# siyi-wind/MDViT

Hardware: NVIDIA B200
Metric: mdvit_train_images_per_sec (higher is better)
Workload: dtype bf16

## Files before the change

include/mdvit_b200.h:

```cpp
#ifndef MDVIT_B200_H
#define MDVIT_B200_H
#include <stdint.h>

#ifdef __cplusplus
extern "C" {
#endif

#define MDV_ACT_NONE 0
#define MDV_ACT_GELU 1
#define MDV_ACT_RELU 2
#define MDV_ACT_HSWISH 3

int mdv_version(void);
long long mdv_launch_count(void);
int mdv_set_pdl(int enabled);

typedef struct MdvGemmEpi {
    const float* bias;
    const float* residual;
    const void* mul_gelu_grad;
    void* out_preact;
    void* out;
    const float* rowscale;
    const void* rng;
// ... 16 lines not shown

int mdv_conv3_gemm(const void* x, int x_f32, int ldx, const void* Wm, int ldw, int B, int H, int W, int Cin, int N, int flip,
                   const MdvGemmEpi* epi, void* stream);

int mdv_conv3_wgrad(const void* dz_bf16, int ldz, const void* x_bf16, int ldx, int B, int H, int W, int Cin, int P, float* dWm, int ldc,
                    void* stream);

int mdv_gemm_tn(const void* A, int lda, const void* B, int ldb, int R, int P, int Q, float* C, int ldc, void* stream);

int mdv_mlp_supported(int C, int hidden);
int mdv_mlp_fwd(const void* a_bf16, const void* w1_bf16, const float* b1, const void* w2_bf16, const float* b2, const float* residual,
                float* out, void* hact_out, void* u_out, int M, int C, int hidden, float drop_p, const void* rng, uint32_t drop_stream1,
                uint32_t drop_stream2, const float* rowscale, int rows_per_scale, void* stream);
int mdv_mlp_bwd(const void* dy_bf16, const void* w2t_bf16, const void* u_bf16, const void* w1t_bf16, void* du_out, float* dx_out,
                float* colsum1, int M, int C, int hidden, void* stream);

int mdv_gemm_tune(int force_bn, int force_stages, int force_split);
int mdv_gemm_force_pair(int mode);

int mdv_layernorm_fwd(const float* x, const float* gamma, const float* beta, float eps, void* y_bf16, float* mean,
                      float* rstd, int M, int C, void* stream);
int mdv_layernorm_bwd(const float* dy, const float* x, const float* mean, const float* rstd, const float* gamma,
                      const float* dres, float* dx, void* dx_masked_bf16, const float* rowscale, int rows_per_scale,
                      float drop_p, const void* rng, uint32_t drop_stream, float* dgamma, float* dbeta,
                      float* dbias_masked , int M, int C, void* stream);

#define MDV_MAX_GROUPS 8
typedef struct MdvPtrTable {
    void* p[MDV_MAX_GROUPS];
} MdvPtrTable;

int mdv_layernorm_fwd_gp(const float* x, MdvPtrTable gamma, MdvPtrTable beta, float eps, void* y_bf16, float* mean, float* rstd,
                         int G, int Mg, int C, void* stream);
int mdv_layernorm_bwd_gp(const float* dy, const float* x, const float* mean, const float* rstd, MdvPtrTable gamma,
                         const float* dres, float* dx, void* dx_masked_bf16, const float* rowscale, int rows_per_scale,
                         float drop_p, const void* rng, uint32_t drop_stream, MdvPtrTable dgamma, MdvPtrTable dbeta,
                         float* dbias_masked, int G, int Mg, int C, void* stream);
int mdv_bn_train_fwd_gp(const float* z, int G, int Mg, int C, float eps, float momentum, MdvPtrTable running_mean,
                        MdvPtrTable running_var, MdvPtrTable num_batches_tracked, MdvPtrTable gamma, MdvPtrTable beta, int act,
                        float* mean, float* rstd, void* y, int y_bf16, void* ws, void* stream);
int mdv_bn_act_bwd_gp(const float* dy, const float* z, const float* mean, const float* rstd, MdvPtrTable gamma, MdvPtrTable beta,
                      int act, void* dz, int dz_bf16, MdvPtrTable dgamma, MdvPtrTable dbeta, int G, int Mg, int C, void* ws,
                      void* stream);

int mdv_bn_stats(const float* z, int M, int C, float eps, float momentum, int training, float* running_mean,
                 float* running_var, long long* num_batches_tracked, float* mean, float* rstd, void* ws, void* stream);
int mdv_bn_fold(const float* gamma, const float* beta, const float* running_mean, const float* running_var, const float* conv_bias,
                float eps, float* scale, float* shift, int C, void* stream);
int mdv_bn_act_fwd(const float* z, const float* mean, const float* rstd, const float* gamma, const float* beta, int act,
                   void* y, int y_bf16, int M, int C, void* stream);
int mdv_bn_act_bwd(const float* dy, const float* z, const float* mean, const float* rstd, const float* gamma,
                   const float* beta, int act, void* dz, int dz_bf16, float* dgamma, float* dbeta, int M, int C, void* ws,
                   void* stream);
int mdv_bn_train_fwd_grouped(const float* z, int G, int Mg, int C, float eps, float momentum, float* running_mean, float* running_var,
                             long long* num_batches_tracked, const float* gamma, const float* beta, int act, float* mean, float* rstd,
                             void* y, int y_bf16, void* ws, void* stream);
int mdv_bn_act_bwd_grouped(const float* dy, const float* z, const float* mean, const float* rstd, const float* gamma, const float* beta,
                           int act, void* dz, int dz_bf16, float* dgamma, float* dbeta, int G, int Mg, int C, void* ws, void* stream);
int mdv_bn_act_bwd_rank1(const float* dlog, const float* wrow, int rows_per_sample, float drop_p, const void* rng,
                         uint32_t drop_stream, const float* z, const float* mean, const float* rstd, const float* gamma,
                         const float* beta, int act, void* dz, int dz_bf16, float* dgamma, float* dbeta, int M, int C, void* ws,
                         void* stream);

int mdv_dwconv3(const float* in, const float* w, const float* bias, void* out, int out_bf16, int B, int Hi, int Wi, int Ho,
                int Wo, int C, int stride, int transposed, int residual, void* stream);
int mdv_dwconv3_wgrad(const float* dy, const float* x, float* dw, float* db, int B, int Hi, int Wi, int Ho, int Wo, int C,
                      int stride, void* stream);
int mdv_gconv2_fwd(const float* skip, const float* up, const float* w, void* out, int out_bf16, int B, int H, int W, int C,
                   void* stream);
int mdv_gconv2_bwd(const float* dout, const float* skip, const float* up, const float* w, float* dskip, float* dup, float* dw,
                   int B, int H, int W, int C, void* stream);
int mdv_im2col3(const void* in, int in_bf16, void* col, int col_bf16, int B, int Hi, int Wi, int Ho, int Wo, int C, int stride,
                int ldc, void* stream);
int mdv_im2col_stem(const float* img_nchw, void* col, int col_bf16, int B, int Hi, int Wi, void* stream);
int mdv_col2im3(const float* dcol, float* dx, int B, int Hi, int Wi, int Ho, int Wo, int C, int stride, int ldc, void* stream);
int mdv_im2col3_dil(const void* in, int in_bf16, void* col, int B, int H, int W, int C, int dil, int ldc, void* stream);
int mdv_col2im3_dil(const float* dcol, float* dx, int B, int H, int W, int C, int dil, int ldc, int accumulate, void* stream);
int mdv_upsample_fwd(const void* in, int in_bf16, int ld_in, void* out, int out_bf16, int ld_out, int B, int Hi, int Wi, int Ho,
                     int Wo, int C, void* stream);
int mdv_upsample_add(float* out, int ld_out, int B, int Ho, int Wo, int C, const float* in0, int H0, int W0, const float* in1, int H1,
                     int W1, const float* in2, int H2, int W2, void* stream);
int mdv_upsample_bwd(const void* dout, int dout_bf16, int ld_out, float* din, int ld_in, int B, int Hi, int Wi, int Ho, int Wo,
                     int C, float* ws, void* stream);

long long mdv_attn_stats_floats(int B, int C, int heads);
long long mdv_attn_ws_floats(int B, int C, int heads);
int mdv_attn_fwd(const void* qkv_bf16, const float* gate, const float* crpe_w3, const float* crpe_b3, const float* crpe_w5,
                 const float* crpe_b5, const float* crpe_w7, const float* crpe_b7, float* stats, float* ws, void* out_bf16,
                 void* e_out_bf16 , int B, int H, int W, int C, int heads,
                 void* stream);
int mdv_attn_bwd(const void* qkv_bf16, const void* dy_bf16, const void* y_bf16, const void* e_bf16, const float* gate, const float* crpe_w3,
                 const float* crpe_b3, const float* crpe_w5, const float* crpe_b5, const float* crpe_w7, const float* crpe_b7,
                 const float* stats, void* dqkv_bf16, float* dgate, float* dcrpe_w3, float* dcrpe_b3, float* dcrpe_w5,
                 float* dcrpe_b5, float* dcrpe_w7, float* dcrpe_b7,
                 float* dbias_qkv , float* ws, int B,
                 int H, int W, int C, int heads,
                 void* stream);
int mdv_da_gate_fwd(const float* label, const float* w1, const float* b1, const float* w2, const float* b2, float* hid_out,
                    float* gate, int B, int nd, int hid, int C, int heads, void* stream);
int mdv_da_gate_bwd(const float* label, const float* w2, const float* hid_in, const float* gate, const float* dgate, float* dw1,
                    float* db1, float* dw2, float* db2, float* ws , int B, int nd, int hid, int C, int heads,
                    void* stream);

int mdv_sdpa_fwd(const void* qkv_bf16, const float* gate, void* out_bf16, float* lse, int B, int N, int C, int heads, float scale,
                 void* stream);
int mdv_sdpa_bwd(const void* qkv_bf16, const float* gate, const void* out_bf16, const float* lse, const void* dout_bf16,
                 void* dqkv_bf16, float* dgate, int B, int N, int C, int heads, float scale, void* stream);

int mdv_im2col_k(const float* in, int in_nchw, void* col, int col_bf16, int B, int Hi, int Wi, int Ho, int Wo, int C, int k, int stride,
                 int pad, int ldc, void* stream);
int mdv_col2im_k(const float* dcol, float* dx, int B, int Hi, int Wi, int Ho, int Wo, int C, int k, int stride, int pad, int ldc,
                 void* stream);
int mdv_maxpool3s2_fwd(const float* in, float* out, void* tap_u8, int B, int Hi, int Wi, int C, void* stream);
int mdv_maxpool3s2_bwd(const float* dout, const void* tap_u8, float* din, int B, int Hi, int Wi, int C, void* stream);
int mdv_add_act(const float* a, const float* b, float* out, long long n, int act, void* stream);
int mdv_relu_bwd(const float* dy, const float* y, float* dx, long long n, void* stream);
int mdv_resize_ac_fwd(const float* in, float* out, int B, int Hi, int Wi, int Ho, int Wo, int C, void* stream);
int mdv_resize_ac_bwd(const float* dout, float* din, int B, int Hi, int Wi, int Ho, int Wo, int C, void* stream);
int mdv_gate_cat_fwd(const float* g, const float* pgate, const float* x, const float* vgate, const float* bp, float* out, int M, int C1,
                     int C2, int C3, int rows_per_sample, void* stream);
int mdv_gate_cat_bwd(const float* dout, const float* g, const float* pgate, const float* x, const float* vgate, float* dg, float* dp, float* dx,
                     float* dv, float* dbp, int M, int C1, int C2, int C3, int rows_per_sample, void* stream);
int mdv_channel_pool_fwd(const float* x, float* out, void* arg_i32, int M, int C, void* stream);
int mdv_channel_pool_bwd(const float* dout, const void* arg_i32, float* dx, int M, int C, void* stream);
int mdv_dropout2d(const float* x, float* out, int M, int C, int rows_per_sample, float p, const void* rng, uint32_t drop_stream, void* stream);
int mdv_structure_weit(const float* mask, float* weit, float* ws, int B, int H, int W, void* stream);
int mdv_structure_loss_fwd(const float* pred, const float* mask, const float* weit, void* sums, float* loss, int B, int HW, void* stream);
int mdv_structure_loss_bwd(const float* pred, const float* mask, const float* weit, const void* sums, const float* gout, float coef,
                           float* dpred, int B, int HW, int accumulate, void* stream);

int mdv_rowdot_fwd(const void* x, int x_bf16, const float* w, const float* bias, float* out, int M, int C, int rows_per_sample,
                   float drop_p, const void* rng, uint32_t drop_stream, void* stream);
int mdv_rowdot_bwd(const float* dlog, const void* x, int x_bf16, const float* w, float* dx, float* dw, float* db, int M, int C,
                   int rows_per_sample, float drop_p, const void* rng, uint32_t drop_stream, void* stream);
int mdv_colsum(const void* x, int x_bf16, int ld, float* out, int M, int C, void* stream);
int mdv_cast_bf16(const float* in, int ld_in, void* out_bf16, int ld_out, long long M, int C, const float* rowscale,
                  int rows_per_scale, float drop_p, const void* rng, uint32_t drop_stream, float* colsum, void* stream);
int mdv_add_f32(const void* in, int in_bf16, int ld_in, float* out, int ld_out, long long M, int C, int accumulate, void* stream);
typedef struct MdvMatmulDesc {
    const float* A;
    const float* B;
    float* C;
    const float* u;
    const float* v;
    int lda, ldb, ldc, M, N, K, trans_a, trans_b, accumulate, pad_;
} MdvMatmulDesc;
int mdv_matmul_f32_grouped(const MdvMatmulDesc* descs, int n, void* stream);
int mdv_prep_weight(const float* src, void* dst, int R, int Cc, int ld, int mode, int cin, void* stream);
typedef struct MdvPrepDesc {
    const float* src;
    void* dst;
    int rows, cols, ld, mode, cin, pad_;
} MdvPrepDesc;
int mdv_prep_weights_batched(const MdvPrepDesc* descs_dev, int n, void* stream);
int mdv_unperm_conv_grad(const float* g, int ld, float* dw, int R, int cin, void* stream);

int mdv_loss_sums(const float* out, const float* aux, const void* label, int label_u8, void* sums, long long n, void* stream);
int mdv_loss_finalize(const void* sums, double n_total, float* losses , void* stream);
int mdv_loss_bwd(const float* out, const float* aux, const void* label, int label_u8, const void* sums, double n_total,
                 const float* coef, float* dout, float* daux, long long n, void* stream);

int mdv_seg_counts(const float* logits, const void* label, int label_u8, void* counts, long long n, void* stream);

int mdv_adamw(float* p, const float* g, float* m, float* v, void* hyper, long long n, void* stream);
int mdv_rng_bump(void* rng , void* stream);
int mdv_droppath_scale(float* scale, int B, float p, const void* rng, uint32_t drop_stream, void* stream);
// ... 6 lines not shown
```

mdvit_b200/csrc/conv.cu:

```cuda
#include "../../include/mdvit_b200.h"
#include "common.cuh"

namespace {

typedef int idx_t;

__device__ __forceinline__ float4 ld4(const float* p) { return *reinterpret_cast<const float4*>(p); }
__device__ __forceinline__ void st4(float* p, float4 v) { *reinterpret_cast<float4*>(p) = v; }
__device__ __forceinline__ void st4(bf16* p, float4 v) {
    *reinterpret_cast<uint2*>(p) = make_uint2(f2_to_bf2(v.x, v.y), f2_to_bf2(v.z, v.w));
}
__device__ __forceinline__ float4 ld4(const bf16* p) {
    uint2 u = *reinterpret_cast<const uint2*>(p);
    float2 a = bf2_to_f2(u.x), b = bf2_to_f2(u.y);
    return make_float4(a.x, a.y, b.x, b.y);
}
__device__ __forceinline__ void fma4(float4& a, const float4& w, const float4& x) {
    a.x += w.x * x.x; a.y += w.y * x.y; a.z += w.z * x.z; a.w += w.w * x.w;
}

template <typename TO, int STRIDE>
__global__ void __launch_bounds__(256) dwconv3_kernel(const float* __restrict__ in, const float* __restrict__ w,
                                                       const float* __restrict__ bias, TO* __restrict__ out, int B, int Hi,
                                                       int Wi, int Ho, int Wo, int C, int stride_rt, int transposed, int residual) {
// ... 866 lines not shown
        const int xa = S * xi - S / 2, ya = S * yi - S / 2;
        float acc[8] = {0.f, 0.f, 0.f, 0.f, 0.f, 0.f, 0.f, 0.f};
#pragma unroll
        for (int r = 0; r < 2 * S; ++r) {
            const int y = min(max(ya + r, 0), Ho - 1);
            const float wy = wty[yi * 2 * S + r];
            const bf16* prow = dout + ((size_t)(b * Ho + y) * Wo) * ld_out + c;
            uint4 v[2 * S];
#pragma unroll
            for (int k = 0; k < 2 * S; ++k) v[k] = *reinterpret_cast<const uint4*>(prow + (size_t)min(max(xa + k, 0), Wo - 1) * ld_out);
#pragma unroll
            for (int k = 0; k < 2 * S; ++k) fma8(acc, wy * wtab[xi * 2 * S + k], v[k]);
        }
        float* o = din + (size_t)pix * ld_in + c;
        st4(o, make_float4(acc[0], acc[1], acc[2], acc[3]));
        st4(o + 4, make_float4(acc[4], acc[5], acc[6], acc[7]));
    }
}

template <int S>
__global__ void __launch_bounds__(256) upsample_bwd_int1_kernel(const float* __restrict__ dout, float* __restrict__ din, int B, int Hi,
                                                                 int Wi) {
    MDV_PDL_SYNC();
    extern __shared__ float wtab[];
    float* wty = wtab + Wi * 2 * S;
    upsample_wtab<S>(wtab, Wi);
    upsample_wtab<S>(wty, Hi);
    __syncthreads();
    const int Ho = Hi * S, Wo = Wi * S;
    const int total = B * Hi * Wi;
    for (int idx = blockIdx.x * blockDim.x + threadIdx.x; idx < total; idx += gridDim.x * blockDim.x) {
        const int xi = idx % Wi;
        const int yi = (idx / Wi) % Hi;
        const int b = idx / (Wi * Hi);
        const int xa = S * xi - S / 2, ya = S * yi - S / 2;
        float wx[2 * S];
#pragma unroll
        for (int k = 0; k < 2 * S; ++k) wx[k] = wtab[xi * 2 * S + k];
        float acc = 0.f;
#pragma unroll 2
        for (int r = 0; r < 2 * S; ++r) {
            const int y = min(max(ya + r, 0), Ho - 1);
            const float* prow = dout + (size_t)(b * Ho + y) * Wo;
            float rs = 0.f;
#pragma unroll
            for (int k = 0; k < 2 * S; ++k) rs = fmaf(wx[k], __ldg(prow + min(max(xa + k, 0), Wo - 1)), rs);
            acc = fmaf(wty[yi * 2 * S + r], rs, acc);
        }
        din[idx] = acc;
    }
}

template <int S>
__global__ void __launch_bounds__(256) upsample_bwd_v_kernel(const float* __restrict__ tmp, float* __restrict__ din, int ld_in, int B,
                                                              int Hi, int Wi, int C) {
    MDV_PDL_SYNC();
    const int Ho = Hi * S;
    const int cvn = C >> 2;
    const float sc = 1.f / S;
    const int total = B * Hi * Wi * cvn;
    for (int idx = blockIdx.x * blockDim.x + threadIdx.x; idx < total; idx += gridDim.x * blockDim.x) {
        const int c = (idx % cvn) * 4;
        const int pix = idx / cvn;
        const int xi = pix % Wi;
        const int yi = (pix / Wi) % Hi;
        const int b = pix / (Wi * Hi);
        const int ya = S * yi - S / 2;
        float4 acc = make_float4(0.f, 0.f, 0.f, 0.f);
#pragma unroll
        for (int r = 0; r < 2 * S; ++r) {
            const int y = ya + r;
            if (y < 0 || y >= Ho) continue;
            int y0, y1;
            float ly;
            bil_src(y, sc, Hi, y0, y1, ly);
            const float wgt = (y0 == yi ? 1.f - ly : 0.f) + (y1 == yi ? ly : 0.f);
            const float4 v = ld4(tmp + ((size_t)(b * Ho + y) * Wi + xi) * C + c);
            acc.x += wgt * v.x; acc.y += wgt * v.y; acc.z += wgt * v.z; acc.w += wgt * v.w;
        }
        st4(din + (size_t)pix * ld_in + c, acc);
    }
}

inline int grid_for(long long total_threads) {
    long long b = (total_threads + 255) / 256;
    const long long cap = (long long)MDV_NUM_SMS * 16;
    return (int)(b < cap ? (b > 0 ? b : 1) : cap);
}
inline bool fits_i32(long long n) { return n > 0 && n < 0x7fffffffLL; }
inline int pix_per_block_for(long long npix, int col_blocks) {
    int want = (8 * MDV_NUM_SMS) / (col_blocks > 0 ? col_blocks : 1);
    if (want < 1) want = 1;
    long long ppb = (npix + want - 1) / want;
    if (ppb < 64) ppb = 64;
    return (int)ppb;
}

}

extern "C" int mdv_dwconv3(const float* in, const float* w, const float* bias, void* out, int out_bf16, int B, int Hi, int Wi,
                           int Ho, int Wo, int C, int stride, int transposed, int residual, void* stream) {
    if (!in || !w || !out || (C & 3) || B <= 0) return MDV_ERR_ARG;
    if (!fits_i32((long long)B * (Hi > Ho ? Hi : Ho) * (Wi > Wo ? Wi : Wo) * C)) return MDV_ERR_UNSUPPORTED;
    const long long total = (long long)B * Ho * Wo * (C / 4);
    const size_t smem = (size_t)10 * C * sizeof(float);
    cudaStream_t st = (cudaStream_t)stream;
    if (stride == 1 && Hi == Ho && Wi == Wo) {
        int seg = Hi >= 64 ? 16 : (Hi >= 16 ? 8 : Hi);
        while (seg < Hi && seg < 64 && (long long)mdv_cdiv((long long)Wi * C, 1024) * mdv_cdiv(Hi, 2 * seg) * B >= 4 * MDV_NUM_SMS) seg *= 2;
        dim3 grid(mdv_cdiv((long long)Wi * C, 1024), mdv_cdiv(Hi, seg), B);
        if (out_bf16) mdv_launch(dwconv3_s1_kernel<bf16>, dim3(grid), dim3(256), 0, st, in, w, bias, (bf16*)out, Hi, Wi, C, transposed, residual, seg);
        else mdv_launch(dwconv3_s1_kernel<float>, dim3(grid), dim3(256), 0, st, in, w, bias, (float*)out, Hi, Wi, C, transposed, residual, seg);
        MDV_CHECK_LAUNCH();
        return MDV_OK;
    }
#define MDV_DW(TO_, S_) mdv_launch((dwconv3_kernel<TO_, S_>), dim3(grid_for(total)), dim3(256), smem, st, in, w, bias, (TO_*)out, B, Hi, Wi, Ho, Wo, C, stride, transposed, residual)
    if (out_bf16) {
        if (stride == 2) MDV_DW(bf16, 2); else if (stride == 1) MDV_DW(bf16, 1); else MDV_DW(bf16, 0);
    } else {
        if (stride == 2) MDV_DW(float, 2); else if (stride == 1) MDV_DW(float, 1); else MDV_DW(float, 0);
    }
#undef MDV_DW
    MDV_CHECK_LAUNCH();
    return MDV_OK;
}

extern "C" int mdv_dwconv3_wgrad(const float* dy, const float* x, float* dw, float* db, int B, int Hi, int Wi, int Ho, int Wo,
                                 int C, int stride, void* stream) {
    if (!dy || !x || !dw || B <= 0) return MDV_ERR_ARG;
    if (!fits_i32((long long)B * Hi * Wi * C)) return MDV_ERR_UNSUPPORTED;
    if (stride == 1 && Hi == Ho && Wi == Wo && !(C & 3) && C * 40 <= 48 * 1024) {
        int seg = Hi >= 64 ? 16 : (Hi >= 16 ? 8 : Hi);
        while (seg < Hi && seg < 64 && (long long)mdv_cdiv((long long)Wi * C, 1024) * mdv_cdiv(Hi, 2 * seg) * B >= 4 * MDV_NUM_SMS) seg *= 2;
        dim3 grid(mdv_cdiv((long long)Wi * C, 1024), mdv_cdiv(Hi, seg), B);
        mdv_launch(dwconv3_s1_wgrad_kernel, dim3(grid), dim3(256), (size_t)C * 10 * sizeof(float), (cudaStream_t)stream, dy, x, dw, db, Hi, Wi, C, seg);
        MDV_CHECK_LAUNCH();
        return MDV_OK;
    }
    const long long npix = (long long)B * Ho * Wo;
    const int cb = mdv_cdiv(C, 32);
    const int ppb = pix_per_block_for(npix, cb);
    dim3 grid(cb, mdv_cdiv(npix, ppb));
    mdv_launch(dwconv3_wgrad_kernel, dim3(grid), dim3(256), 0, (cudaStream_t)stream, dy, x, dw, db, B, Hi, Wi, Ho, Wo, C, stride, ppb);
    MDV_CHECK_LAUNCH();
    return MDV_OK;
}

extern "C" int mdv_gconv2_fwd(const float* skip, const float* up, const float* w, void* out, int out_bf16, int B, int H, int W, int C,
                              void* stream) {
    if (!skip || !up || !w || !out || (C & 3)) return MDV_ERR_ARG;
    if (!fits_i32((long long)B * H * W * C)) return MDV_ERR_UNSUPPORTED;
    {
        const int seg = H >= 64 ? 16 : (H >= 16 ? 8 : H);
        if (out_bf16)
            mdv_launch(gconv2_s_fwd_kernel<bf16>, dim3(mdv_cdiv(W * (C / 2), 256), mdv_cdiv(H, seg), B), dim3(256), 0, (cudaStream_t)stream, skip, up, w,
                       (bf16*)out, H, W, C, seg);
        else
            mdv_launch(gconv2_s_fwd_kernel<float>, dim3(mdv_cdiv(W * (C / 2), 256), mdv_cdiv(H, seg), B), dim3(256), 0, (cudaStream_t)stream, skip, up, w,
                       (float*)out, H, W, C, seg);
    }
    MDV_CHECK_LAUNCH();
    return MDV_OK;
}

extern "C" int mdv_gconv2_bwd(const float* dout, const float* skip, const float* up, const float* w, float* dskip, float* dup,
                              float* dw, int B, int H, int W, int C, void* stream) {
// ... 116 lines not shown
                                int H1, int W1, const float* in2, int H2, int W2, void* stream) {
    if (!out || B <= 0 || Ho <= 0 || Wo <= 0 || C <= 0 || (C & 3) || (ld_out & 3) || ld_out < C || (reinterpret_cast<uintptr_t>(out) & 15))
        return MDV_ERR_ARG;
    UpIn3 in = {};
    int n = 0;
    const float* ps[3] = {in0, in1, in2};
    const int hs[3] = {H0, H1, H2}, ws[3] = {W0, W1, W2};
    for (int k = 0; k < 3; ++k) {
        if (!ps[k]) continue;
        if (hs[k] <= 0 || ws[k] <= 0 || (reinterpret_cast<uintptr_t>(ps[k]) & 15)) return MDV_ERR_ARG;
        if (!fits_i32((long long)B * hs[k] * ws[k] * C)) return MDV_ERR_UNSUPPORTED;
        in.p[n] = ps[k]; in.H[n] = hs[k]; in.W[n] = ws[k];
        ++n;
    }
    if (!n) return MDV_OK;
    const int seg = Ho >= 64 ? 32 : Ho;
    mdv_launch(upsample_add_kernel, dim3(mdv_cdiv(Wo * (C / 4), 256), mdv_cdiv(Ho, seg), B), dim3(256), 0, (cudaStream_t)stream, in, n, out,
               ld_out, Ho, Wo, C, seg);
    MDV_CHECK_LAUNCH();
    return MDV_OK;
}

extern "C" int mdv_upsample_bwd(const void* dout, int dout_bf16, int ld_out, float* din, int ld_in, int B, int Hi, int Wi, int Ho,
                                int Wo, int C, float* ws, void* stream) {
    if (!dout || !din || B <= 0) return MDV_ERR_ARG;
    if (!fits_i32((long long)B * Ho * Wo * (ld_out > C ? ld_out : C))) return MDV_ERR_UNSUPPORTED;
    cudaStream_t st = (cudaStream_t)stream;
    if (C == 1) {
        if (dout_bf16) return MDV_ERR_UNSUPPORTED;
        const int S1 = (Ho % Hi == 0 && Wo % Wi == 0 && Ho / Hi == Wo / Wi) ? Ho / Hi : 0;
        if ((S1 == 2 || S1 == 4 || S1 == 8) && (size_t)(Wi + Hi) * 2 * S1 * sizeof(float) <= 40 * 1024) {
            const dim3 g1(grid_for((long long)B * Hi * Wi));
            const size_t sm = (size_t)(Wi + Hi) * 2 * S1 * sizeof(float);
            if (S1 == 2) mdv_launch(upsample_bwd_int1_kernel<2>, g1, dim3(256), sm, st, (const float*)dout, din, B, Hi, Wi);
            else if (S1 == 4) mdv_launch(upsample_bwd_int1_kernel<4>, g1, dim3(256), sm, st, (const float*)dout, din, B, Hi, Wi);
            else mdv_launch(upsample_bwd_int1_kernel<8>, g1, dim3(256), sm, st, (const float*)dout, din, B, Hi, Wi);
            MDV_CHECK_LAUNCH();
            return MDV_OK;
        }
        mdv_launch((upsample_bwd_kernel<float, 1>), dim3(grid_for((long long)B * Hi * Wi)), dim3(256), 0, st, (const float*)dout, 1, din, 1, B, Hi, Wi, Ho, Wo, 1);
        MDV_CHECK_LAUNCH();
        return MDV_OK;
    }
    if ((C & 3) || (ld_in & 3) || (ld_out & 3)) return MDV_ERR_ARG;
    const int g = grid_for((long long)B * Hi * Wi * (C / 4));
    const int S = (Ho % Hi == 0 && Wo % Wi == 0 && Ho / Hi == Wo / Wi) ? Ho / Hi : 0;
    if (ws && (S == 4 || S == 8) && fits_i32((long long)B * Ho * Wi * C)) {
        const int gh = grid_for((long long)B * Ho * Wi * (C / 4));
        const bool v8 = dout_bf16 && !(C & 7) && !(ld_out & 7) && !(reinterpret_cast<uintptr_t>(dout) & 15);
        const int gh8 = grid_for((long long)B * Ho * Wi * (C / 8));
#define MDV_UPH(SS)                                                                                                                  \
    if (v8) mdv_launch((upsample_bwd_h8_kernel<SS>), dim3(gh8), dim3(256), (size_t)Wi * 2 * SS * sizeof(float), st, (const bf16*)dout, ld_out, ws, B, Ho, Wi, C); \
    else if (dout_bf16) mdv_launch((upsample_bwd_h_kernel<bf16, SS>), dim3(gh), dim3(256), 0, st, (const bf16*)dout, ld_out, ws, B, Ho, Wi, C);     \
    else mdv_launch((upsample_bwd_h_kernel<float, SS>), dim3(gh), dim3(256), 0, st, (const float*)dout, ld_out, ws, B, Ho, Wi, C);             \
    MDV_CHECK_LAUNCH();                                                                                                              \
    mdv_launch((upsample_bwd_v_kernel<SS>), dim3(g), dim3(256), 0, st, (const float*)ws, din, ld_in, B, Hi, Wi, C);
        if (S == 4) { MDV_UPH(4) } else { MDV_UPH(8) }
#undef MDV_UPH
        MDV_CHECK_LAUNCH();
        return MDV_OK;
    }
    if (S == 2 && dout_bf16 && !(C & 7) && !(ld_out & 7) && !(ld_in & 3) && !(reinterpret_cast<uintptr_t>(dout) & 15)) {
        mdv_launch(upsample_bwd_int8x2_kernel, dim3(grid_for((long long)B * Hi * Wi * (C / 8))), dim3(256), (size_t)(Wi + Hi) * 4 * sizeof(float), st,
                   (const bf16*)dout, ld_out, din, ld_in, B, Hi, Wi, C);
        MDV_CHECK_LAUNCH();
        return MDV_OK;
    }
    if ((S == 2 || S == 4 || S == 8) && (long long)B * Hi * Wi * (C / 4) < 0x7fffffffLL) {
#define MDV_UPB(SS)                                                                                                              \
    if (dout_bf16) mdv_launch((upsample_bwd_int_kernel<bf16, SS>), dim3(g), dim3(256), 0, st, (const bf16*)dout, ld_out, din, ld_in, B, Hi, Wi, C);     \
    else mdv_launch((upsample_bwd_int_kernel<float, SS>), dim3(g), dim3(256), 0, st, (const float*)dout, ld_out, din, ld_in, B, Hi, Wi, C);
        if (S == 2) { MDV_UPB(2) } else if (S == 4) { MDV_UPB(4) } else { MDV_UPB(8) }
#undef MDV_UPB
        MDV_CHECK_LAUNCH();
        return MDV_OK;
    }
    if (dout_bf16)
        mdv_launch((upsample_bwd_kernel<bf16, 4>), dim3(g), dim3(256), 0, st, (const bf16*)dout, ld_out, din, ld_in, B, Hi, Wi, Ho, Wo, C);
    else
        mdv_launch((upsample_bwd_kernel<float, 4>), dim3(g), dim3(256), 0, st, (const float*)dout, ld_out, din, ld_in, B, Hi, Wi, Ho, Wo, C);
    MDV_CHECK_LAUNCH();
    return MDV_OK;
}
```

mdvit_b200/ops.py:

```python
import ctypes
import itertools
import weakref

import torch

from . import _lib as L
from ._lib import ACT_GELU, ACT_HSWISH, ACT_NONE, ACT_RELU, GemmEpi, check, ptr, ptr_table

BF16, F32 = torch.bfloat16, torch.float32
HEADS = 8

_rng_state = {}
_stream_counter = itertools.count(1)


def rng_tensor(device):
    t = _rng_state.get(device)
    if t is None:
        t = torch.tensor([0x5EED, 0], dtype=torch.int64, device=device)
        _rng_state[device] = t
    return t


def manual_seed(seed, device):
# ... 205 lines not shown
        global _BN_GROUPS
        self.prev, _BN_GROUPS = _BN_GROUPS, self.g

    def __exit__(self, *exc):
        global _BN_GROUPS
        _BN_GROUPS = self.prev


def current_bn_groups():
    return _BN_GROUPS


def bn_fold(weight, bias, running_mean, running_var, conv_bias=None, eps=1e-5):
    C = weight.numel()
    st = torch.empty((2, C), dtype=F32, device=weight.device)
    check(L.lib().mdv_bn_fold(ptr(weight), ptr(bias), ptr(running_mean), ptr(running_var), ptr(conv_bias), ctypes.c_float(eps), ptr(st[0]),
                              ptr(st[1]), C, L.stream()), "mdv_bn_fold")
    return st[0], st[1]


def bn_forward(z, M, C, weight, bias, running_mean, running_var, nbt, training, act, out_bf16, eps=1e-5, momentum=0.1):
    dev = z.device
    G = _BN_GROUPS if training else 1
    if M % G:
        raise ValueError("BatchNorm groups must divide the batch")
    Mg = M // G
    z = z.view(M, C)
    mean = torch.empty((G, C), dtype=F32, device=dev)
    rstd = torch.empty((G, C), dtype=F32, device=dev)
    y = torch.empty((M, C), dtype=BF16 if out_bf16 else F32, device=dev)
    if isinstance(weight, list):
        if not training or len(weight) != G:
            raise ValueError("per-group BatchNorm parameter sets need train mode and one set per bn_groups() group")
        ws = torch.empty(2 * C * G, dtype=torch.float64, device=dev)
        check(L.lib().mdv_bn_train_fwd_gp(ptr(z), G, Mg, C, ctypes.c_float(eps), ctypes.c_float(momentum), ptr_table(running_mean),
                                          ptr_table(running_var), ptr_table(nbt), ptr_table(weight), ptr_table(bias), act, ptr(mean), ptr(rstd),
                                          ptr(y), int(out_bf16), ptr(ws), L.stream()), "mdv_bn_train_fwd_gp")
        return y, mean, rstd
    if training:
        ws = torch.empty(2 * C * G, dtype=torch.float64, device=dev)
        check(L.lib().mdv_bn_train_fwd_grouped(ptr(z), G, Mg, C, ctypes.c_float(eps), ctypes.c_float(momentum), ptr(running_mean),
                                               ptr(running_var), ptr(nbt), ptr(weight), ptr(bias), act, ptr(mean), ptr(rstd), ptr(y),
                                               int(out_bf16), ptr(ws), L.stream()), "mdv_bn_train_fwd_grouped")
        return y, mean, rstd
    check(L.lib().mdv_bn_stats(ptr(z), M, C, ctypes.c_float(eps), ctypes.c_float(momentum), 0, ptr(running_mean), ptr(running_var), ptr(nbt),
                               ptr(mean[0]), ptr(rstd[0]), None, L.stream()), "mdv_bn_stats")
    check(L.lib().mdv_bn_act_fwd(ptr(z), ptr(mean[0]), ptr(rstd[0]), ptr(weight), ptr(bias), act, ptr(y), int(out_bf16), M, C, L.stream()),
          "mdv_bn_act_fwd")
    return y, mean, rstd


def bn_backward(dy, z, mean, rstd, weight, bias, act, M, C, dz_bf16=True):
    dev = z.device
    G = mean.shape[0]
    Mg = M // G
    dy, z = dy.view(M, C), z.view(M, C)
    dz = torch.empty((M, C), dtype=BF16 if dz_bf16 else F32, device=dev)
    ws = torch.empty(3 * C * G, dtype=torch.float64, device=dev)
    if isinstance(weight, list):
        tg, tb = [gtarget(w) for w in weight], [gtarget(b) for b in bias]
        check(L.lib().mdv_bn_act_bwd_gp(ptr(dy), ptr(z), ptr(mean), ptr(rstd), ptr_table(weight), ptr_table(bias), act, ptr(dz), int(dz_bf16),
                                        ptr_table([t[0] for t in tg]), ptr_table([t[0] for t in tb]), G, Mg, C, ptr(ws), L.stream()),
              "mdv_bn_act_bwd_gp")
        return dz, [t[1] for t in tg], [t[1] for t in tb]
    dg, rg = gtarget(weight)
    db, rb = gtarget(bias)
    check(L.lib().mdv_bn_act_bwd_grouped(ptr(dy), ptr(z), ptr(mean), ptr(rstd), ptr(weight), ptr(bias), act, ptr(dz), int(dz_bf16), ptr(dg),
                                         ptr(db), G, Mg, C, ptr(ws), L.stream()), "mdv_bn_act_bwd_grouped")
    return dz, rg, rb


def upsample_fwd(x, out, B, Hi, Wi, Ho, Wo, C, ld_in=None, ld_out=None):
    check(L.lib().mdv_upsample_fwd(ptr(x), int(x.dtype == BF16), ld_in or C, ptr(out), int(out.dtype == BF16), ld_out or C, B, Hi, Wi,
                                   Ho, Wo, C, L.stream()), "mdv_upsample_fwd")
    return out


def upsample_bwd(dout, B, Hi, Wi, Ho, Wo, C, ld_out=None):
    din = torch.empty((B * Hi * Wi, C), dtype=F32, device=dout.device)
    ws = torch.empty(B * Ho * Wi * C, dtype=F32, device=dout.device) if (C >= 64 and Ho == Wo and Hi == Wi and Ho // Hi in (4, 8) and Ho % Hi == 0) else None
    check(L.lib().mdv_upsample_bwd(ptr(dout), int(dout.dtype == BF16), ld_out or C, ptr(din), C, B, Hi, Wi, Ho, Wo, C, ptr(ws), L.stream()),
          "mdv_upsample_bwd")
    return din


def upsample_add(out, ins, B, Ho, Wo, C, ld_out=None):
    args = []
    for x, Hi, Wi in list(ins) + [(None, 0, 0)] * (3 - len(ins)):
        args += [ptr(x), Hi, Wi]
    check(L.lib().mdv_upsample_add(ptr(out), ld_out or C, B, Ho, Wo, C, *args, L.stream()), "mdv_upsample_add")
    return out


class _MatmulDesc(ctypes.Structure):
    _fields_ = [("A", ctypes.c_void_p), ("B", ctypes.c_void_p), ("C", ctypes.c_void_p), ("u", ctypes.c_void_p), ("v", ctypes.c_void_p)] + \
               [(n, ctypes.c_int) for n in ("lda", "ldb", "ldc", "M", "N", "K", "trans_a", "trans_b", "accumulate", "pad_")]


def mm(A, B, C, M, N, K, *, lda=None, ldb=None, ldc=None, trans_a=False, trans_b=False, accumulate=False, u=None, v=None):
    if C is None:
        return None
    d = _MatmulDesc(ptr(A), ptr(B), ptr(C), ptr(u), ptr(v), lda or (M if trans_a else K), ldb or (K if trans_b else N), ldc or N, M, N, K,
                    int(trans_a), int(trans_b), int(accumulate), 0)
    d.tensors = (A, B, C, u, v)
    return d


def matmul_f32(problems):
    ds = [d for d in problems if d is not None]
    if ds:
        check(L.lib().mdv_matmul_f32_grouped((_MatmulDesc * len(ds))(*ds), len(ds), L.stream()), "mdv_matmul_f32_grouped")


def _contig(t):
    return t if t.is_contiguous() else t.contiguous()


_BWD_MODE = "all"


class backward_mode:
    def __init__(self, mode):
        assert mode in ("all", "da_only")
        self.mode = mode

    def __enter__(self):
        global _BWD_MODE
        self.prev, _BWD_MODE = _BWD_MODE, self.mode

    def __exit__(self, *exc):
        global _BWD_MODE
        _BWD_MODE = self.prev


def wgrad_on():
    return _BWD_MODE == "all"


_FWD_TAG = None
_FWD_USE_CB = None
_GRAD_READY_CB = None


def set_forward_tag(tag):
    global _FWD_TAG
    _FWD_TAG = tag


def set_forward_use_cb(cb):
    global _FWD_USE_CB
    _FWD_USE_CB = cb


def set_grad_ready_cb(cb):
    global _GRAD_READY_CB
    _GRAD_READY_CB = cb


def _fwd_mark(ctx):
    ctx.tag = _FWD_TAG
    if _FWD_USE_CB is not None:
        _FWD_USE_CB(_FWD_TAG, ctx.params)


def _grads_done(ctx):
    if _GRAD_READY_CB is not None:
# ... 871 lines not shown
        Cs = [t.shape[2] for t in xs]
        C1 = Cs[0]
        Kx = C1 + C5
        rm, rv, nb = bufs
        lib = L.lib()
        lw, lb = (l1w, l2w, l3w, l4w), (l1b, l2b, l3b, l4b)
        with _dev_ctx(x1):
            w1x = torch.empty((hc, Kx), dtype=F32, device=dev)
            if C5:
                check(lib.mdv_add_f32(ptr(fw[:, 4 * hc:]), 0, K, ptr(w1x[:, C1:]), Kx, hc, C5, 0, L.stream()), "mdv_add_f32")
            wps = [torch.empty((hc, Cs[i]), dtype=F32, device=dev) for i in range(1, 4)]
            cb = torch.empty((4, hc), dtype=F32, device=dev)
            check(lib.mdv_add_f32(ptr(fb), 0, hc, ptr(cb), hc, 1, hc, 0, L.stream()), "mdv_add_f32")
            matmul_f32([mm(fw, lw[0], w1x, hc, C1, hc, lda=K, ldc=Kx)] +
                       [mm(fw[:, i * hc:], lw[i], wps[i - 1], hc, Cs[i], hc, lda=K) for i in range(1, 4)] +
                       [mm(fw[:, i * hc:], lb[i], cb[i], hc, 1, hc, lda=K, accumulate=i == 0) for i in range(4)])
            xa = torch.empty((M0, Kx), dtype=BF16, device=dev)
            cast_bf16(xs[0], M0, C1, out=xa, ld_out=Kx)
            if C5:
                cast_bf16(x5, M0, C5, out=xa[:, C1:], ld_out=Kx)
            z = torch.empty((M0, hc), dtype=F32, device=dev)
            gemm_nt(xa, cast_bf16(w1x, hc, Kx), M0, hc, Kx, z, bias=cb[0])
            acts, ys = [xa], []
            for i in range(1, 4):
                Hi, Wi = sizes[i]
                Mi, Ci = B * Hi * Wi, Cs[i]
                a = cast_bf16(xs[i], Mi, Ci)
                acts.append(a)
                ys.append((gemm_nt(a, cast_bf16(wps[i - 1], hc, Ci), Mi, hc, Ci, torch.empty((Mi, hc), dtype=F32, device=dev), bias=cb[i]), Hi, Wi))
            upsample_add(z, ys, B, H, W, hc)
            a5, mean, rstd = bn_forward(z, M0, hc, g, b, rm, rv, nb, training, ACT_RELU, True)
            p2 = drop2d if training else 0.0
            sid = new_stream_id() if p2 > 0 else 0
            lo = torch.empty(M0, dtype=F32, device=dev)
            check(lib.mdv_rowdot_fwd(ptr(a5), 1, ptr(ow), ptr(ob), ptr(lo), M0, hc, H * W, ctypes.c_float(p2),
                                     ptr(rng_tensor(dev)) if p2 > 0 else None, sid, L.stream()), "mdv_rowdot_fwd")
            out = upsample_fwd(lo, torch.empty((B, 1, Ho, Wo), dtype=F32, device=dev), B, H, W, Ho, Wo, 1)
            if training:
                wts = [_bf16_t(w1x, hc, Kx)] + [_bf16_t(wps[i - 1], hc, Cs[i]) for i in range(1, 4)]
            else:
                wts, z = [], None
        ctx.save_for_backward(z, mean, rstd, a5, *acts, *wts)
        ctx.params = (l1w, l1b, l2w, l2b, l3w, l3b, l4w, l4b, fw, fb, g, b, ow, ob)
        ctx.meta = (B, sizes, Ho, Wo, hc, K, C5, p2, sid, training, Cs)
        _fwd_mark(ctx)
        return out

    @staticmethod
    def backward(ctx, dout):
        B, sizes, Ho, Wo, hc, K, C5, p2, sid, training, Cs = ctx.meta
        if not training:
            raise RuntimeError("mdvit_b200: backward through eval-mode BatchNorm is not supported")
        z, mean, rstd, a5, *rest = ctx.saved_tensors
        acts, wts = rest[:4], rest[4:]
        l1w, l1b, l2w, l2b, l3w, l3b, l4w, l4b, fw, fb, g, b, ow, ob = ctx.params
        (H, W) = sizes[0]
        M0, dev = B * H * W, dout.device
        C1 = Cs[0]
        Kx = C1 + C5
        lib = L.lib()
        dout = _contig(dout.float())
        lw, lb = (l1w, l2w, l3w, l4w), (l1b, l2b, l3b, l4b)
        with _dev_ctx(dout):
            dlo = upsample_bwd(dout, B, H, W, Ho, Wo, 1)
            g_ow, r_ow = gtarget(ow)
            g_ob, r_ob = gtarget(ob)
            if g_ow is not None:
                check(lib.mdv_rowdot_bwd(ptr(dlo), ptr(a5), 1, ptr(ow), None, ptr(g_ow), ptr(g_ob), M0, hc, H * W, ctypes.c_float(p2),
                                         ptr(rng_tensor(dev)) if p2 > 0 else None, sid, L.stream()), "mdv_rowdot_bwd")
            dz = torch.empty((M0, hc), dtype=BF16, device=dev)
            ws_bn = torch.empty(3 * hc + (B * hc + 1) // 2, dtype=torch.float64, device=dev)
            g_g, rg = gtarget(g)
            g_b, rb = gtarget(b)
            check(lib.mdv_bn_act_bwd_rank1(ptr(dlo), ptr(ow), H * W, ctypes.c_float(p2), ptr(rng_tensor(dev)) if p2 > 0 else None, sid,
                                           ptr(z), ptr(mean), ptr(rstd), ptr(g), ptr(b), ACT_RELU, ptr(dz), 1, ptr(g_g), ptr(g_b), M0, hc,
                                           ptr(ws_bn), L.stream()), "mdv_bn_act_bwd_rank1")
            g_fw, r_fw = gtarget(fw, (hc, K))
            g_fb, r_fb = gtarget(fb)
            tw = [gtarget(lw[i], (hc, Cs[i])) for i in range(4)]
            tb = [gtarget(lb[i]) for i in range(4)]
            wgrad = any(t is not None for t in [g_fw, g_fb] + [t[0] for t in tw + tb])
            gx = [gemm_nt(dz, wts[0], M0, C1, hc, torch.empty((B, H * W, C1), dtype=F32, device=dev))]
            dx5 = gemm_nt(dz, wts[0][C1:], M0, C5, hc, torch.empty((B, H * W, C5), dtype=F32, device=dev)) if C5 else None
            if wgrad:
                s = colsum(dz, M0, hc, torch.zeros(hc, dtype=F32, device=dev))
                Es = [gemm_tn(dz, acts[0], M0, hc, Kx, torch.zeros((hc, Kx), dtype=F32, device=dev))]
            for i in range(1, 4):
                Hi, Wi = sizes[i]
                Mi, Ci = B * Hi * Wi, Cs[i]
                dzi = cast_bf16(upsample_bwd(dz, B, Hi, Wi, H, W, hc), Mi, hc)
                gx.append(gemm_nt(dzi, wts[i], Mi, Ci, hc, torch.empty((B, Hi * Wi, Ci), dtype=F32, device=dev)))
                if wgrad:
                    Es.append(gemm_tn(dzi, acts[i], Mi, hc, Ci, torch.zeros((hc, Ci), dtype=F32, device=dev)))
            if wgrad:
                probs = []
                for i in range(4):
                    Ci, ldE = Cs[i], (Kx if i == 0 else Cs[i])
                    wf = fw[:, i * hc:]
                    gwf = g_fw[:, i * hc:] if g_fw is not None else None
                    probs += [mm(Es[i], lw[i], gwf, hc, hc, Ci, lda=ldE, ldc=K, trans_b=True, accumulate=True, u=s, v=lb[i]),
                              mm(wf, Es[i], tw[i][0], hc, Ci, hc, lda=K, ldb=ldE, trans_a=True, accumulate=True),
                              mm(wf, s, tb[i][0], hc, 1, hc, lda=K, trans_a=True, accumulate=True)]
                matmul_f32(probs)
                if g_fw is not None and C5:
                    check(lib.mdv_add_f32(ptr(Es[0][:, C1:]), 0, Kx, ptr(g_fw[:, 4 * hc:]), K, hc, C5, 1, L.stream()), "mdv_add_f32")
                if g_fb is not None:
                    check(lib.mdv_add_f32(ptr(s), 0, hc, ptr(g_fb), hc, 1, hc, 1, L.stream()), "mdv_add_f32")
        _grads_done(ctx)
        return (gx[0], gx[1], gx[2], gx[3], dx5, tw[0][1], tb[0][1], tw[1][1], tb[1][1], tw[2][1], tb[2][1], tw[3][1], tb[3][1], r_fw,
                r_fb, rg, rb, r_ow, r_ob, None, None, None, None, None, None)


class SplitDomainsFn(torch.autograd.Function):

    @staticmethod
    def forward(ctx, x, G):
        B = x.shape[0] // G
        ctx.G, ctx.shape_b = G, (B,) + tuple(x.shape[1:])
        return tuple(x.narrow(0, g * B, B) for g in range(G))

    @staticmethod
    def backward(ctx, *grads):
        ref = next(g for g in grads if g is not None)
        parts = [g if g is not None else torch.zeros(ctx.shape_b, dtype=ref.dtype, device=ref.device) for g in grads]
        return torch.cat(parts, dim=0), None


def _label_arg(label):
    if label.dtype == torch.uint8:
        return _contig(label), 1
    return _contig(label.float()), 0


class SegLossFn(torch.autograd.Function):

    @staticmethod
    def forward(ctx, n_total, reduce_sums, G, *tensors):
        outs = [_contig(t.float()) for t in tensors[:G]]
        auxs = [(_contig(t.float()) if t is not None else None) for t in tensors[G:2 * G]]
        labs = [_label_arg(t) for t in tensors[2 * G:3 * G]]
        dev = outs[0].device
        lib = L.lib()
        with _dev_ctx(outs[0]):
            sums = torch.empty((G, 8), dtype=torch.float64, device=dev)
            for g in range(G):
                check(lib.mdv_loss_sums(ptr(outs[g]), ptr(auxs[g]), ptr(labs[g][0]), labs[g][1], ptr(sums[g]), outs[g].numel(), L.stream()),
                      "mdv_loss_sums")
            if reduce_sums is not None:
                reduce_sums(sums)
            losses = torch.empty((G, 3), dtype=F32, device=dev)
            nt = [float(n_total or o.numel()) for o in outs]
            for g in range(G):
                check(lib.mdv_loss_finalize(ptr(sums[g]), ctypes.c_double(nt[g]), ptr(losses[g]), L.stream()), "mdv_loss_finalize")
        ctx.save_for_backward(sums, *outs, *[a for a in auxs if a is not None], *[l for l, _ in labs])
        ctx.G, ctx.nt, ctx.has_aux, ctx.lab_u8 = G, nt, [a is not None for a in auxs], [u for _, u in labs]
        return losses

    @staticmethod
    def backward(ctx, dl):
        G = ctx.G
        sums, *rest = ctx.saved_tensors
        outs, rest = rest[:G], rest[G:]
        na = sum(ctx.has_aux)
        it = iter(rest[:na])
        auxs = [next(it) if h else None for h in ctx.has_aux]
        labs = rest[na:]
        lib = L.lib()
        dl = _contig(dl.float())
        douts, dauxs = [], []
        with _dev_ctx(outs[0]):
            for g in range(G):
                dout = torch.empty_like(outs[g])
                daux = torch.empty_like(auxs[g]) if auxs[g] is not None else None
# ... 428 lines not shown
```

Before: 2363.

## Fuse three-level bilinear upsample backward and column sum into one pyramid kernel

```diff
diff --git a/include/mdvit_b200.h b/include/mdvit_b200.h
--- a/include/mdvit_b200.h
+++ b/include/mdvit_b200.h
@@ -122,6 +122,8 @@
                      int W1, const float* in2, int H2, int W2, void* stream);
 int mdv_upsample_bwd(const void* dout, int dout_bf16, int ld_out, float* din, int ld_in, int B, int Hi, int Wi, int Ho, int Wo,
                      int C, float* ws, void* stream);
+int mdv_upsample_bwd_pyramid(const void* dz, int ld, void* dz2, void* dz3, void* dz4, float* s, int B, int Ho, int Wo, int C, int H2,
+                             int W2, int H3, int W3, int H4, int W4, void* stream);
 
 long long mdv_attn_stats_floats(int B, int C, int heads);
 long long mdv_attn_ws_floats(int B, int C, int heads);
diff --git a/mdvit_b200/csrc/conv.cu b/mdvit_b200/csrc/conv.cu
--- a/mdvit_b200/csrc/conv.cu
+++ b/mdvit_b200/csrc/conv.cu
@@ -972,6 +972,110 @@
     }
 }
 
+template <int S>
+__device__ __forceinline__ void pyr_flush(float* sm, float4 a, int Wo, int CG, bf16* __restrict__ out_row, int C) {
+    st4(sm + threadIdx.x * 4, a);
+    __syncthreads();
+    const int Wi = Wo / S;
+    if ((int)threadIdx.x < Wi * CG) {
+        const int xi = threadIdx.x / CG, g = threadIdx.x - xi * CG;
+        float4 acc = make_float4(0.f, 0.f, 0.f, 0.f);
+#pragma unroll 2
+        for (int k = 0; k < 2 * S; ++k) {
+            const int x = S * xi - S / 2 + k;
+            if (x < 0 || x >= Wo) continue;
+            int x0, x1;
+            float lx;
+            bil_src(x, 1.f / S, Wi, x0, x1, lx);
+            const float w = (x0 == xi ? 1.f - lx : 0.f) + (x1 == xi ? lx : 0.f);
+            const float4 p = ld4(sm + (x * CG + g) * 4);
+            acc.x += w * p.x; acc.y += w * p.y; acc.z += w * p.z; acc.w += w * p.w;
+        }
+        *reinterpret_cast<uint2*>(out_row + (size_t)xi * C + g * 4) = make_uint2(f2_to_bf2(acc.x, acc.y), f2_to_bf2(acc.z, acc.w));
+    }
+    __syncthreads();
+}
+
+template <int S>
+__device__ __forceinline__ void pyr_row(float4& a0, float4& a1, int& r, float4 v, int y, int Ho, int Wo, int CG, int lo, int hi,
+                                        float* sm, bf16* __restrict__ out_img, int C) {
+    int i0, i1;
+    float ly;
+    bil_src(y, 1.f / S, Ho / S, i0, i1, ly);
+    if (i0 > r) {
+        if (r >= lo && r < hi) pyr_flush<S>(sm, a0, Wo, CG, out_img + (size_t)r * (Wo / S) * C, C);
+        a0 = a1;
+        a1 = make_float4(0.f, 0.f, 0.f, 0.f);
+        ++r;
+    }
+    const float w0 = (1.f - ly) + (i1 == r ? ly : 0.f);
+    const float w1 = i1 != r ? ly : 0.f;
+    a0.x += w0 * v.x; a0.y += w0 * v.y; a0.z += w0 * v.z; a0.w += w0 * v.w;
+    a1.x += w1 * v.x; a1.y += w1 * v.y; a1.z += w1 * v.z; a1.w += w1 * v.w;
+}
+
+constexpr int PYR_RING = 8;
+
+__global__ void __launch_bounds__(256, 4) upsample_bwd_pyramid_kernel(const bf16* __restrict__ dz, int ld, bf16* __restrict__ o2,
+                                                                    bf16* __restrict__ o3, bf16* __restrict__ o4, float* __restrict__ s,
+                                                                    int Ho, int Wo, int C, int CG, int NB) {
+    MDV_PDL_SYNC();
+    __shared__ __align__(16) float sm[256 * 4];
+    __shared__ __align__(16) uint2 ring[PYR_RING][256];
+    const int x = threadIdx.x / CG, g = threadIdx.x - x * CG;
+    const int b = blockIdx.y, c0 = blockIdx.x * CG * 4;
+    const bf16* src = dz + ((size_t)b * Ho * Wo + x) * ld + c0 + g * 4;
+    const size_t row_pitch = (size_t)Wo * ld;
+    bf16* out2 = o2 + (size_t)b * (Ho / 2) * (Wo / 2) * C + c0;
+    bf16* out3 = o3 + (size_t)b * (Ho / 4) * (Wo / 4) * C + c0;
+    bf16* out4 = o4 + (size_t)b * (Ho / 8) * (Wo / 8) * C + c0;
+    const int band = blockIdx.z * 8 * NB;
+    const int own_end = min(Ho, band + 8 * NB);
+    const int y_beg = max(0, band - 4), y_end = min(Ho, own_end + 4);
+    const uint32_t ring_s = (uint32_t)__cvta_generic_to_shared(&ring[0][threadIdx.x]);
+    auto fetch = [&](int y) {
+        if (y < y_end)
+            asm volatile("cp.async.ca.shared.global [%0], [%1], 8;" ::"r"(ring_s + (uint32_t)((y % PYR_RING) * 256 * sizeof(uint2))),
+                         "l"(src + (size_t)y * row_pitch) : "memory");
+        asm volatile("cp.async.commit_group;" ::: "memory");
+    };
+#pragma unroll
+    for (int j = 0; j < PYR_RING - 1; ++j) fetch(y_beg + j);
+    const float4 zero = make_float4(0.f, 0.f, 0.f, 0.f);
+    float4 a2 = zero, b2 = zero, a3 = zero, b3 = zero, a4 = zero, b4 = zero, cs = zero;
+    int r2, r3, r4, i1;
+    float l;
+    bil_src(y_beg, 0.5f, Ho / 2, r2, i1, l);
+    bil_src(y_beg, 0.25f, Ho / 4, r3, i1, l);
+    bil_src(y_beg, 0.125f, Ho / 8, r4, i1, l);
+    const int lo2 = band / 2, hi2 = own_end / 2, lo3 = band / 4, hi3 = own_end / 4, lo4 = band / 8, hi4 = own_end / 8;
+#pragma unroll 1
+    for (int y = y_beg; y < y_end; ++y) {
+        fetch(y + PYR_RING - 1);
+        asm volatile("cp.async.wait_group %0;" ::"n"(PYR_RING - 1) : "memory");
+        const uint2 raw = ring[y % PYR_RING][threadIdx.x];
+        const float2 lo = bf2_to_f2(raw.x), hi = bf2_to_f2(raw.y);
+        const float4 v = make_float4(lo.x, lo.y, hi.x, hi.y);
+        if (y >= band && y < own_end) { cs.x += v.x; cs.y += v.y; cs.z += v.z; cs.w += v.w; }
+        pyr_row<2>(a2, b2, r2, v, y, Ho, Wo, CG, lo2, hi2, sm, out2, C);
+        pyr_row<4>(a3, b3, r3, v, y, Ho, Wo, CG, lo3, hi3, sm, out3, C);
+        pyr_row<8>(a4, b4, r4, v, y, Ho, Wo, CG, lo4, hi4, sm, out4, C);
+    }
+    if (r2 >= lo2 && r2 < hi2) pyr_flush<2>(sm, a2, Wo, CG, out2 + (size_t)r2 * (Wo / 2) * C, C);
+    if (r3 >= lo3 && r3 < hi3) pyr_flush<4>(sm, a3, Wo, CG, out3 + (size_t)r3 * (Wo / 4) * C, C);
+    if (r4 >= lo4 && r4 < hi4) pyr_flush<8>(sm, a4, Wo, CG, out4 + (size_t)r4 * (Wo / 8) * C, C);
+    if (s) {
+        st4(sm + threadIdx.x * 4, cs);
+        __syncthreads();
+        const int CH = CG * 4;
+        if ((int)threadIdx.x < CH) {
+            float t = 0.f;
+            for (int xx = 0; xx < Wo; ++xx) t += sm[xx * CH + threadIdx.x];
+            atomicAdd(s + c0 + threadIdx.x, t);
+        }
+    }
+}
+
 inline int grid_for(long long total_threads) {
     long long b = (total_threads + 255) / 256;
     const long long cap = (long long)MDV_NUM_SMS * 16;
@@ -1254,3 +1358,18 @@
     MDV_CHECK_LAUNCH();
     return MDV_OK;
 }
+
+extern "C" int mdv_upsample_bwd_pyramid(const void* dz, int ld, void* dz2, void* dz3, void* dz4, float* s, int B, int Ho, int Wo, int C,
+                                        int H2, int W2, int H3, int W3, int H4, int W4, void* stream) {
+    auto mis16 = [](const void* p) { return (reinterpret_cast<uintptr_t>(p) & 15) != 0; };
+    if (!dz || !dz2 || !dz3 || !dz4 || B <= 0 || Ho <= 0 || Wo <= 0 || C <= 0 || (C & 7) || (ld & 7) || ld < C) return MDV_ERR_ARG;
+    if (H2 * 2 != Ho || W2 * 2 != Wo || H3 * 4 != Ho || W3 * 4 != Wo || H4 * 8 != Ho || W4 * 8 != Wo) return MDV_ERR_ARG;
+    if (mis16(dz) || mis16(dz2) || mis16(dz3) || mis16(dz4)) return MDV_ERR_ARG;
+    if (Wo > 256 || B > 65535) return MDV_ERR_UNSUPPORTED;
+    const int CG = (!(C & 15) && Wo * 4 <= 256) ? 4 : (Wo * 2 <= 256 ? 2 : 1);
+    const int NB = 2;
+    mdv_launch(upsample_bwd_pyramid_kernel, dim3(C / (4 * CG), B, mdv_cdiv(H4, NB)), dim3(Wo * CG), 0, (cudaStream_t)stream, (const bf16*)dz,
+               ld, (bf16*)dz2, (bf16*)dz3, (bf16*)dz4, s, Ho, Wo, C, CG, NB);
+    MDV_CHECK_LAUNCH();
+    return MDV_OK;
+}
diff --git a/mdvit_b200/ops.py b/mdvit_b200/ops.py
--- a/mdvit_b200/ops.py
+++ b/mdvit_b200/ops.py
@@ -311,6 +311,19 @@
     check(L.lib().mdv_upsample_bwd(ptr(dout), int(dout.dtype == BF16), ld_out or C, ptr(din), C, B, Hi, Wi, Ho, Wo, C, ptr(ws), L.stream()),
           "mdv_upsample_bwd")
     return din
+
+
+def pyramid_sizes_ok(Ho, Wo, C, sizes):
+    return (C % 8 == 0 and Ho % 8 == 0 and Wo % 8 == 0 and Wo <= 256 and
+            [tuple(hw) for hw in sizes] == [(Ho // f, Wo // f) for f in (2, 4, 8)])
+
+
+def upsample_bwd_pyramid(dz, B, Ho, Wo, C, sizes, s=None, ld=None):
+    outs = [torch.empty((B * h * w, C), dtype=BF16, device=dz.device) for h, w in sizes]
+    (h2, w2), (h3, w3), (h4, w4) = sizes
+    check(L.lib().mdv_upsample_bwd_pyramid(ptr(dz), ld or C, *[ptr(t) for t in outs], ptr(s), B, Ho, Wo, C, h2, w2, h3, w3, h4, w4,
+                                           L.stream()), "mdv_upsample_bwd_pyramid")
+    return outs
 
 
 def upsample_add(out, ins, B, Ho, Wo, C, ld_out=None):
@@ -1348,13 +1361,18 @@
             wgrad = any(t is not None for t in [g_fw, g_fb] + [t[0] for t in tw + tb])
             gx = [gemm_nt(dz, wts[0], M0, C1, hc, torch.empty((B, H * W, C1), dtype=F32, device=dev))]
             dx5 = gemm_nt(dz, wts[0][C1:], M0, C5, hc, torch.empty((B, H * W, C5), dtype=F32, device=dev)) if C5 else None
+            pyr = pyramid_sizes_ok(H, W, hc, sizes[1:])
+            s = torch.zeros(hc, dtype=F32, device=dev) if wgrad else None
+            if pyr:
+                dzs = upsample_bwd_pyramid(dz, B, H, W, hc, sizes[1:], s)
+            elif wgrad:
+                colsum(dz, M0, hc, s)
             if wgrad:
-                s = colsum(dz, M0, hc, torch.zeros(hc, dtype=F32, device=dev))
                 Es = [gemm_tn(dz, acts[0], M0, hc, Kx, torch.zeros((hc, Kx), dtype=F32, device=dev))]
             for i in range(1, 4):
                 Hi, Wi = sizes[i]
                 Mi, Ci = B * Hi * Wi, Cs[i]
-                dzi = cast_bf16(upsample_bwd(dz, B, Hi, Wi, H, W, hc), Mi, hc)
+                dzi = dzs[i - 1] if pyr else cast_bf16(upsample_bwd(dz, B, Hi, Wi, H, W, hc), Mi, hc)
                 gx.append(gemm_nt(dzi, wts[i], Mi, Ci, hc, torch.empty((B, Hi * Wi, Ci), dtype=F32, device=dev)))
                 if wgrad:
                     Es.append(gemm_tn(dzi, acts[i], Mi, hc, Ci, torch.zeros((hc, Ci), dtype=F32, device=dev)))
```

New measurement: 2372 (median of 6 runs). Within noise of the previous version (+0.4%).
